# skim0119/gym-softrobot

Hardware: AMD Instinct MI355X
Metric: env_steps_per_sec (higher is better)
Workload: dtype f64

## Files before the change

### gym_softrobot_amd/_capi.py

```python
from __future__ import annotations

import ctypes as C
import os
from pathlib import Path

ABI_VERSION = 17

FEAT_GRAVITY = 1 << 0
FEAT_POINT_FORCE_NODE0_X = 1 << 1
FEAT_PENDULUM_BC = 1 << 2
FEAT_ANALYTICAL_DAMPER = 1 << 3
FEAT_FIXED_BC = 1 << 4
FEAT_TIP_FORCE = 1 << 5
FEAT_MOVING_BASE_BC = 1 << 6
FEAT_LAPLACE_FILTER = 1 << 7
FEAT_PLANE_CONTACT_ANISO = 1 << 8
FEAT_REST_KAPPA_ACTION = 1 << 9
FEAT_OCTO_HEAD = 1 << 10
FEAT_SPLINE_MUSCLE_TORQUES = 1 << 11
FEAT_SUCKER_CONSTRAINT = 1 << 12
FEAT_COOMM_MUSCLES = 1 << 13
MAX_SUCKERS = 4
MAX_MUSCLES = 4
MUSCLE_LONGITUDINAL = 0
# ... 893 lines not shown

_VP = C.c_void_p
_EXPORTS = {
    "softrod_abi_version": (C.c_int, []),
    "softrod_source_hash": (C.c_char_p, []),
    "softrod_action_dim": (C.c_int, [C.c_int]),
    "softrod_obs_dim": (C.c_int, [C.c_int]),
    "softrod_aux_dim": (C.c_int, [C.c_int]),
    "softrod_config_softpendulum": (C.c_int, [C.POINTER(SoftrodConfig), C.c_int]),
    "softrod_config_softpendulum3d": (C.c_int, [C.POINTER(SoftrodConfig), C.c_int]),
    "softrod_config_arm_single": (C.c_int, [C.POINTER(SoftrodConfig), C.c_int]),
    "softrod_config_octo_flat": (C.c_int, [C.POINTER(SoftrodConfig), C.c_int]),
    "softrod_config_soft_arm": (C.c_int, [C.POINTER(SoftrodConfig), C.c_int]),
    "softrod_config_arm_push": (C.c_int, [C.POINTER(SoftrodConfig), C.c_int, C.c_int]),
    "softrod_config_arm_pull_weight": (C.c_int, [C.POINTER(SoftrodConfig), C.c_int]),
    "softrod_config_muscle_octopus": (C.c_int, [C.POINTER(SoftrodConfig), C.c_int, C.c_int]),
    "softrod_set_muscle_layers": (C.c_int, [_VP, _VP, _VP]),
    "softrod_set_spline_table": (C.c_int, [_VP, _VP, _VP]),
    "softrod_config_action_dim": (C.c_int, [C.POINTER(SoftrodConfig)]),
    "softrod_config_obs_dim": (C.c_int, [C.POINTER(SoftrodConfig)]),
    "softrod_reset_octo": (C.c_int, [_VP, _VP, _VP, _VP, _VP, _VP]),
    "softrod_autoreset_enable": (C.c_int, [_VP, C.c_int]),
    "softrod_autoreset_same_step": (C.c_int, [_VP, C.c_int]),
    "softrod_final_view": (C.c_int, [_VP, C.POINTER(C.c_void_p), C.POINTER(C.c_void_p), C.POINTER(C.c_void_p)]),
    "softrod_queue_push": (C.c_int, [_VP, _VP, _VP, C.c_int, _VP]),
    "softrod_queue_push_straight": (C.c_int, [_VP, _VP, _VP, _VP, _VP, C.c_int, _VP]),
    "softrod_queue_push_octo": (C.c_int, [_VP, _VP, _VP, _VP, _VP, C.c_int, _VP]),
    "softrod_queue_status": (C.c_int, [_VP, _VP, _VP, _VP]),
    "softrod_queue_status_begin": (C.c_int, [_VP, _VP]),
    "softrod_queue_status_poll": (C.c_int, [_VP, C.c_int, _VP, _VP]),
    "softrod_queue_advance": (C.c_int, [_VP, _VP, _VP]),
    "softrod_set_action_basis": (C.c_int, [_VP, _VP]),
    "softrod_set_radius_profile": (C.c_int, [_VP, _VP]),
    "softrod_create": (C.c_int, [C.POINTER(SoftrodConfig), C.c_int, C.POINTER(C.c_void_p)]),
    "softrod_reset": (C.c_int, [_VP, _VP, _VP, _VP]),
    "softrod_reset_straight": (C.c_int, [_VP, _VP, _VP, _VP, _VP, _VP]),
    "softrod_step": (C.c_int, [_VP, _VP, _VP, _VP, _VP, _VP, _VP, _VP]),
    "softrod_step_packed": (C.c_int, [_VP, _VP, _VP, _VP, _VP]),
    "softrod_scatter_rows": (C.c_int, [_VP, _VP, _VP, C.c_int, C.c_int, C.c_int64, C.c_int64, C.c_uint32, _VP]),
    "softrod_exchange_alloc": (C.c_int, [C.c_int, C.c_uint64, C.POINTER(C.c_void_p), _VP, C.POINTER(C.c_int)]),
    "softrod_exchange_open": (C.c_int, [C.c_int, _VP, C.c_int, C.POINTER(C.c_void_p)]),
    "softrod_exchange_close": (C.c_int, [C.c_int, _VP]),
    "softrod_exchange_free": (C.c_int, [C.c_int, _VP]),
    "softrod_observe": (C.c_int, [_VP, _VP, _VP, _VP]),
    "softrod_rod_energies": (C.c_int, [_VP, _VP, _VP]),
    "softrod_ground_reaction": (C.c_int, [_VP, _VP, _VP]),
# ... 88 lines not shown
```

### gym_softrobot_amd/backend.py

```python
from __future__ import annotations

import ctypes as C
from typing import Dict, Optional, Tuple

import numpy as np
import torch

from . import _capi
from ._capi import LANE_STRIDE, SoftrodConfig, SoftrodStateView, check, load_library
from .diagnostics import (JointLoads, MuscleLoads, RodClearance, RodDynamics, RodStrains, joint_loads_views,
                          muscle_loads_views, rod_clearance_views, rod_dynamics_views, rod_strains_views)


class _DevArray:

    def __init__(self, ptr: int, shape, typestr: str, owner):
        self._owner = owner
        self.__cuda_array_interface__ = {
            "shape": tuple(shape),
            "typestr": typestr,
            "data": (int(ptr), False),
            "version": 2,
            "strides": None,
        }
# ... 232 lines not shown
        check(
            self._lib.softrod_reset_octo(
                self._h, pos.ctypes.data, dirs.ctypes.data, tg.ctypes.data,
                m.ctypes.data if m is not None else None, self._stream(),
            ),
            self._h,
        )

    def autoreset_enable(self, depth: int) -> None:
        check(self._lib.softrod_autoreset_enable(self._h, int(depth)), self._h)
        self.queue_depth = int(depth)

    def autoreset_same_step(self, on: bool = True) -> None:
        check(self._lib.softrod_autoreset_same_step(self._h, int(bool(on))), self._h)
        self.same_step = bool(on)
        if on and getattr(self, "final_obs", None) is None:
            fo, ft, fa = C.c_void_p(), C.c_void_p(), C.c_void_p()
            check(self._lib.softrod_final_view(self._h, C.byref(fo), C.byref(ft), C.byref(fa)), self._h)
            n = self.n_envs
            self.final_obs = torch.as_tensor(_DevArray(fo.value, (n, self.obs_dim), "<f4", self), device=self.device)
            self.final_time = torch.as_tensor(_DevArray(ft.value, (n,), "<f8", self), device=self.device)
            self.final_aux = torch.as_tensor(_DevArray(fa.value, (n,), "<f8", self), device=self.device)

    @staticmethod
    def _counts(counts, n):
        return np.ascontiguousarray(counts, dtype=np.int32).reshape(n)

    def queue_push(self, theta0, counts) -> None:
        th = np.ascontiguousarray(theta0, dtype=np.float64).reshape(self.n_envs, -1)
        c = self._counts(counts, self.n_envs)
        check(self._lib.softrod_queue_push(self._h, th.ctypes.data, c.ctypes.data, th.shape[1], self._stream()),
              self._h)

    def queue_push_straight(self, start, direction, normal, counts) -> None:
        arrs = [np.ascontiguousarray(v, dtype=np.float64).reshape(self.n_envs, -1, 3)
                for v in (start, direction, normal)]
        c = self._counts(counts, self.n_envs)
        check(self._lib.softrod_queue_push_straight(
            self._h, arrs[0].ctypes.data, arrs[1].ctypes.data, arrs[2].ctypes.data, c.ctypes.data,
            arrs[0].shape[1], self._stream()), self._h)

    def queue_push_octo(self, targets, counts) -> None:
        na = int(self.cfg.n_arm)
        tg = np.ascontiguousarray(targets, dtype=np.float64).reshape(self.n_envs, -1, 4 if self.is_mocto else 2)
        m = tg.shape[1]
        pos, dirs = self._arm_frames()
# ... 351 lines not shown
```

### gym_softrobot_amd/csrc/softrod_capi.hip

```cpp
#include <hip/hip_runtime.h>
#include <hip/hip_ext.h>

#include <cmath>
#include <cstdio>
#include <cstdlib>
#include <cstring>
#include <new>
#include <string>
#include <vector>

#include "softrod_kernels.hpp"
#include "softrod_dynamics_readout.hpp"
#include "softrod_copy_envs.hpp"
#include "softrod_shape.hpp"
#include "softrod_reset_shapes.hpp"

using namespace softrod;

template <class Row>
struct EnvTable {
    Row* dev = nullptr;
    Row* host = nullptr;
    hipEvent_t ev = nullptr;
    void release() {
// ... 36 lines not shown
    std::vector<hipEvent_t> ev_start, ev_stop;
    int timed = 0;
    hipEvent_t ev_reset = nullptr;
    int q_depth = 0;
    double* d_queue = nullptr;
    double* h_queue = nullptr;
    int* d_consumed = nullptr;
    int* d_produced = nullptr;
    int* d_underflow = nullptr;
    uint8_t* d_flags = nullptr;
    int* h_produced = nullptr;
    std::vector<int> seen_consumed;
    std::vector<int2> pending;
    double* h_stage = nullptr;
    int2* h_where = nullptr;
    double* d_stage = nullptr;
    int2* d_where = nullptr;
    size_t stage_cap = 0;
    int* h_status = nullptr;
    hipEvent_t ev_status = nullptr;
    bool status_pending = false;
    hipEvent_t ev_queue = nullptr;
    bool same_step = false;
    float* d_final_obs = nullptr;
    double* d_final_time = nullptr;
    double* d_final_aux = nullptr;
    int rs_count = 0;
    unsigned long long rs_seed = 0;
    double* d_rs_field[4] = {nullptr, nullptr, nullptr, nullptr};
    int* d_rs_index = nullptr;
    int* d_rs_episode = nullptr;
    uint8_t* d_rs_picked = nullptr;
    EnvTable<EnvMaterial> env_mat;
    EnvTable<EnvContact> env_contact;
    int2* d_pairs = nullptr;
    int2* h_pairs = nullptr;
    hipEvent_t ev_pairs = nullptr;
    std::vector<uint8_t> is_dst;
    std::string err;
};

namespace {

thread_local std::string g_err;

int fail(softrod_handle* h, int code, const std::string& msg) {
// ... 238 lines not shown
    }
    SR_HIP(h, hipGetLastError());
    return SOFTROD_OK;
}

enum : unsigned { kOptMuscles = SOFTROD_FEAT_COOMM_MUSCLES, kOptEarlyTerm = kFeatEarlyTerm, kOptEnvMaterial = kFeatEnvMaterial,
                  kOptEnvContact = kFeatEnvContact, kOptCompiledFor = kOptEarlyTerm | kOptEnvMaterial | kOptEnvContact };
constexpr int kAny = -1, kMoctoEnvs = -2;
constexpr unsigned kAnyFeatures = kRuntimeFeatures;
using StepKernel = void (*)(RodParams, StatePtrs, const float*, float*, double*, uint8_t*, uint8_t*, double*, int, int, int);
using OctoKernel = void (*)(RodParams, StatePtrs, const float*, float*, double*, uint8_t*, uint8_t*, int, int, int);
using WindowKernel = void (*)(RodParams, StatePtrs, const float*, int, int);

struct StepRow {
    unsigned feats;
    int env;
    int math, epl;
    int taper, zup;
    int nw_min, nw_max;
    bool windowed;
    unsigned needs, honours;
    StepKernel step; OctoKernel octo; WindowKernel window;
    int epb, waves;
    const char* label;
};

constexpr StepRow compiled_row(unsigned F, int env, int epl, int taper, int nw_min, int nw_max, const char* label) {
    const bool rt = F == kRuntimeFeatures;
    StepRow r{};
    r.feats = rt ? kAnyFeatures : F & ~(kFeatPlaneZup | kOptCompiledFor);
    r.env = env; r.math = SOFTROD_MATH_FAST; r.epl = epl; r.taper = taper; r.nw_min = nw_min; r.nw_max = nw_max;
    r.zup = rt ? kAny : (F & kFeatPlaneZup) != 0;
    r.needs = rt ? 0u : F & kOptCompiledFor;
    r.honours = rt ? 0u : F & (kOptCompiledFor | kOptMuscles);
    r.epb = 1; r.label = label;
    return r;
}
template <unsigned F, int E, int EPL, bool TAPER = false>
constexpr StepRow fast_row(const char* label) {
    StepRow r = compiled_row(F, E, EPL, TAPER, 1, 1, label);
    r.step = softrod_step_fast_kernel<F, E, EPL, TAPER>;
    return r;
}
template <unsigned F, int MAXW, int EPB>
constexpr StepRow octo_row(int env, int nw_min, int nw_max, const char* label) {
    StepRow r = compiled_row(F, env, 1, kAny, nw_min, nw_max, label);
    r.octo = softrod_octo_step_kernel<F, MAXW, EPB>;
    r.epb = EPB; r.waves = EPB == 1 ? 0 : MAXW * EPB;
    return r;
}
template <unsigned F, int RPB>
constexpr StepRow window_row(const char* label) {
    StepRow r = compiled_row(F, SOFTROD_ENV_ARM_SINGLE, 2, 0, 1, 1, label);
    r.window = softrod_step_window_kernel<F, RPB>;
    r.windowed = true; r.epb = RPB; r.waves = 2 * RPB;
    return r;
}
template <bool ET>
constexpr StepRow libm_row(unsigned feats, int env, int zup, int taper, unsigned honours) {
    StepRow r{};
    r.feats = feats; r.env = env; r.math = SOFTROD_MATH_LIBM; r.epl = 1; r.taper = taper; r.zup = zup;
    r.nw_min = r.nw_max = r.epb = 1;
    r.needs = ET ? kOptEarlyTerm : 0u; r.honours = r.needs | kOptMuscles | honours;
    r.step = softrod_step_libm_kernel<ET>;
// ... 105 lines not shown
               "and on SOFTROD_ENV_ARM_PULL_WEIGHT only; other feature mixes: SOFTROD_MATH_LIBM";
    if (opts & kOptEnvMaterial) return material_why_not(h);
    if (opts & kOptEnvContact) return contact_why_not(h);
    return nullptr;
}

struct StepChoice { const StepRow* row; const char* why; };
StepChoice select_step(const softrod_handle* h, int epilogue = 1, unsigned with = 0u) {
    const unsigned opts = active_options(h) | with;
    const int e = h->cfg.env_kind, zup = (h->P.features & kFeatPlaneZup) != 0;
    const bool windowed = h->window_refresh > 0 && epilogue;
    for (const StepRow& r : kStepRows)
        if (r.math == h->cfg.math_mode && (r.feats == kAnyFeatures || r.feats == h->cfg.features) &&
            (r.env == kAny || (r.env == kMoctoEnvs ? mocto_kind(e) : r.env == e)) && r.epl == h->epl &&
            (r.taper == kAny || r.taper == (int)h->tapered) && (r.zup == kAny || r.zup == zup) &&
            r.nw_min <= h->nw && h->nw <= r.nw_max && r.windowed == windowed &&
            (!r.window || r.epb == (h->window_paired ? 4 : 1)) && !(r.needs & ~opts) && !(opts & ~r.honours))
            return {&r, nullptr};
    const char* why = why_no_row(h, with);
    if (!why) why = why_no_row(h, opts);
    return {nullptr, why ? why : "no step kernel is compiled for this handle's feature set, env kind and options"};
}

template <int W, class Row, class Bad, class Build>
int set_env_table(softrod_handle* h, EnvTable<Row>& T, const Row*& slot, unsigned option, const char* what,
                  const double* values, const double (&own)[W], const uint8_t* mask, void* stream, Bad bad, Build build) {
    const StepChoice serves = select_step(h, 1, option);
    if (!serves.row) return fail(h, SOFTROD_EINVAL, serves.why);
    const size_t N = (size_t)h->cfg.n_envs;
    for (size_t i = 0; i < N; ++i) {
        if (mask && !mask[i]) continue;
        if (const char* why = bad(values + W * i)) return fail(h, SOFTROD_EINVAL, what + std::to_string(i) + why);
    }
    SR_ON_DEVICE(h);
    hipStream_t st = (hipStream_t)stream;
    if (!T.dev) {
        SR_HIP(h, hipMalloc((void**)&T.dev, N * sizeof(Row)));
        SR_HIP(h, hipHostMalloc((void**)&T.host, N * sizeof(Row), hipHostMallocDefault));
        SR_HIP(h, hipEventCreateWithFlags(&T.ev, hipEventDisableTiming));
        Row R0;
        build(own, R0);
        for (size_t i = 0; i < N; ++i) T.host[i] = R0;
        slot = T.dev;
        SR_HIP(h, hipMemcpy(h->d_state, &h->S, sizeof(StatePtrs), hipMemcpyHostToDevice));
    } else {
        SR_HIP(h, hipEventSynchronize(T.ev));
    }
    for (size_t i = 0; i < N; ++i)
        if (!mask || mask[i]) build(values + W * i, T.host[i]);
    SR_HIP(h, hipMemcpyAsync(T.dev, T.host, N * sizeof(Row), hipMemcpyHostToDevice, st));
    SR_HIP(h, hipEventRecord(T.ev, st));
    return SOFTROD_OK;
}

template <class K, class... A>
void launch_stamped(K kernel, const dim3& grid, const dim3& block, hipStream_t st, hipEvent_t t0, hipEvent_t t1, A... args) {
    if (t0 || t1) hipExtLaunchKernelGGL(kernel, grid, block, 0, st, t0, t1, 0, args...);
    else hipLaunchKernelGGL(kernel, grid, block, 0, st, args...);
}

int launch_step(softrod_handle* h, const float* actions, float* obs, double* reward,
                uint8_t* term, uint8_t* trunc, double* aux, int n_sub, int epilogue, int pack,
                hipStream_t st) {
    if (h->q_depth > 0 && epilogue && !h->same_step) {
        if (const int rc = launch_autoreset(h, obs, reward, term, trunc, aux, pack, st)) return rc;
        if (h->rs_count > 0)
            if (const int rc = launch_reset_shapes(h, kPickSkipped, nullptr, obs, term, trunc, aux, pack, st)) return rc;
    }
    if ((h->cfg.features & SOFTROD_FEAT_COOMM_MUSCLES) && h->cfg.math_mode == SOFTROD_MATH_FAST) {
        const bool push = h->cfg.env_kind == SOFTROD_ENV_ARM_PUSH || is_pull(h) || is_mocto(h);
        if (is_mocto(h) && (!h->tapered || !h->muscles_set || (h->cfg.env_kind == SOFTROD_ENV_ARM_TWO && !h->basis_set)))
            return fail(h, SOFTROD_EINVAL, "the muscle octopus needs softrod_set_radius_profile and softrod_set_muscle_layers "
                                           "(and SOFTROD_ENV_ARM_TWO softrod_set_action_basis) before it steps");
        if (push && !h->tapered)
            return fail(h, SOFTROD_EINVAL, "SOFTROD_ENV_ARM_PUSH (SOFTROD_MATH_FAST): call softrod_set_radius_profile first "
                                           "(the reference's arm is tapered, arm_push_env.py:160-179)");
        if (!push && h->tapered)
            return fail(h, SOFTROD_EINVAL, "a tapered muscle rod outside SOFTROD_ENV_ARM_PUSH runs under SOFTROD_MATH_LIBM only");
    }
    const StepChoice c = select_step(h, epilogue);
    if (!c.row) return fail(h, SOFTROD_EINVAL, c.why);
    const StepChoice after = c.row->windowed ? select_step(h, 0) : StepChoice{nullptr, nullptr};
    if (c.row->windowed && !after.row) return fail(h, SOFTROD_EINVAL, after.why);
    auto launch = [&](const StepRow& r, int n, int epi, hipEvent_t t0, hipEvent_t t1) {
        const dim3 grid((unsigned)((h->cfg.n_envs + r.epb - 1) / r.epb)), block(kLanes * (r.waves ? r.waves : h->nw));
        if (r.window) launch_stamped(r.window, grid, block, st, t0, t1, h->P, h->S, actions, n, h->window_refresh);
        else if (r.octo) launch_stamped(r.octo, grid, block, st, t0, t1, h->P, h->S, actions, obs, reward, term, trunc, n, epi, pack);
        else launch_stamped(r.step, grid, block, st, t0, t1, h->P, h->S, actions, obs, reward, term, trunc, aux, n, epi, pack);
    };
    const bool timing = h->timed < (int)h->ev_start.size();
    const hipEvent_t t0 = timing ? h->ev_start[h->timed] : nullptr, t1 = timing ? h->ev_stop[h->timed] : nullptr;
    const bool mocto = c.row->env == kMoctoEnvs;
    const bool action_first = mocto && epilogue && actions, epilogue_last = mocto && epilogue;
    const dim3 grid((unsigned)h->cfg.n_envs), block(kLanes * h->nw);
    if (action_first)
        launch_stamped(softrod_mocto_action_kernel, grid, block, st, t0, nullptr, h->P, h->S, actions, n_sub);
    launch(*c.row, n_sub, epilogue, action_first ? nullptr : t0, (after.row || epilogue_last) ? nullptr : t1);
    if (after.row) launch(*after.row, 0, 1, nullptr, epilogue_last ? nullptr : t1);
    if (epilogue_last)
        launch_stamped(softrod_mocto_epilogue_kernel, grid, block, st, nullptr, t1, h->P, h->S, obs, reward, term, trunc, 1, pack);
    SR_HIP(h, hipGetLastError());
    if (timing) ++h->timed;
    if (h->q_depth > 0 && epilogue && h->same_step) {
        if (const int rc = launch_autoreset_same_step(h, obs, aux, pack, st)) return rc;
        if (h->rs_count > 0)
            if (const int rc = launch_reset_shapes(h, kPickFinished, nullptr, obs, term, trunc, aux, pack, st)) return rc;
    }
    return SOFTROD_OK;
}

int upload_and_reset(softrod_handle* h, hipStream_t st, bool use_mask) {
    const size_t N = (size_t)h->cfg.n_envs;
    SR_HIP(h, hipMemcpyAsync(h->d_init, h->h_init, N * h->init_stride * sizeof(double), hipMemcpyHostToDevice, st));
    if (use_mask)
        SR_HIP(h, hipMemcpyAsync(h->d_mask, h->h_mask, N, hipMemcpyHostToDevice, st));
    ResetArgs A{h->d_init, use_mask ? h->d_mask : nullptr};
    if (is_octo(h)) {
        OctoResetArgs OA{h->d_init, h->d_init + N * (size_t)h->cfg.n_arm * 18, use_mask ? h->d_mask : nullptr};
        hipLaunchKernelGGL(softrod_octo_reset_kernel, dim3((unsigned)N), dim3(kLanes * h->nw), 0, st, h->P, h->S, OA);
    } else
// ... 720 lines not shown
        autoreset_release(h);
        h->err = why;
    }
    return rc;
}

int softrod_autoreset_same_step(softrod_handle* h, int on) {
    if (!h) return fail(h, SOFTROD_EINVAL, "null argument");
    if (!h->q_depth) return fail(h, SOFTROD_EINVAL, "call softrod_autoreset_enable first");
    SR_ON_DEVICE(h);
    if (on && !h->d_final_obs) {
        const size_t N = (size_t)h->cfg.n_envs;
        float* fo = nullptr;
        double *ft = nullptr, *fa = nullptr;
        SR_HIP(h, alloc_owned(h, fo, N * (size_t)softrod_config_obs_dim(&h->cfg) * sizeof(float)));
        SR_HIP(h, alloc_owned(h, ft, N * sizeof(double)));
        SR_HIP(h, alloc_owned(h, fa, N * sizeof(double)));
        h->d_final_obs = fo; h->d_final_time = ft; h->d_final_aux = fa;
    }
    h->same_step = on != 0;
    return SOFTROD_OK;
}

int softrod_final_view(softrod_handle* h, float** final_obs, double** final_time, double** final_aux) {
    if (!h || !final_obs || !final_time || !final_aux) return fail(h, SOFTROD_EINVAL, "null argument");
    if (!h->same_step) return fail(h, SOFTROD_EINVAL, "call softrod_autoreset_same_step first");
    *final_obs = h->d_final_obs;
    *final_time = h->d_final_time;
    *final_aux = h->d_final_aux;
    return SOFTROD_OK;
}

namespace {
int queue_begin(softrod_handle* h, const int32_t* counts, int max_count) {
    if (!h->q_depth) return fail(h, SOFTROD_EINVAL, "call softrod_autoreset_enable first");
    if (!counts || max_count < 0) return fail(h, SOFTROD_EINVAL, "bad argument");
    const int N = h->cfg.n_envs;
    for (int e = 0; e < N; ++e) {
        if (counts[e] < 0 || counts[e] > max_count) return fail(h, SOFTROD_EINVAL, "counts[e] out of range");
        if (h->h_produced[e] + counts[e] - h->seen_consumed[e] > h->q_depth)
            return fail(h, SOFTROD_EINVAL, "reset queue overflow: staged + new records exceed depth");
    }
    SR_HIP(h, hipEventSynchronize(h->ev_queue));
    return SOFTROD_OK;
}
double* queue_slot(softrod_handle* h, int e, int k) {
// ... 848 lines not shown
int softrod_last_kernel_ms(softrod_handle* h, float* ms) {
    if (!h || !ms) return fail(h, SOFTROD_EINVAL, "null argument");
    if (h->timed < 1) return fail(h, SOFTROD_EINVAL, "timing not enabled or no timed launch yet");
    SR_ON_DEVICE(h);
    SR_HIP(h, hipEventSynchronize(h->ev_stop[h->timed - 1]));
    SR_HIP(h, hipEventElapsedTime(ms, h->ev_start[h->timed - 1], h->ev_stop[h->timed - 1]));
    return SOFTROD_OK;
}

const char* softrod_last_error(softrod_handle* h) { return h ? h->err.c_str() : g_err.c_str(); }

const char* softrod_kernel_tier(softrod_handle* h) {
    if (!h) return "";
    const StepChoice c = select_step(h);
    std::string t = c.row ? c.row->label : std::string("none: ") + c.why;
    auto fill = [&t](const char* token, const std::string& with) {
        const size_t at = t.find(token);
        if (at != std::string::npos) t.replace(at, std::strlen(token), with);
    };
    fill("{waves}", std::to_string(h->nw) + (h->nw == 1 ? " wave" : " waves"));
    fill("{refresh}", std::to_string(h->window_refresh));
    if (c.row && c.row->windowed)
        if (const StepRow* after = select_step(h, 0).row) t += std::string(" + ") + after->label + " epilogue";
    if (h->env_mat.dev) t += ",env material";
    if (h->env_contact.dev) t += ",env contact";
    h->tier = t;
    return h->tier.c_str();
}

int softrod_destroy(softrod_handle* h) {
    if (!h) return SOFTROD_OK;
    DeviceGuard guard_(h->device);
    (void)hipDeviceSynchronize();
    autoreset_release(h);
    for (void* p : h->owned) (void)hipFree(p);
    for (double* p : h->d_rs_field) if (p) (void)hipFree(p);
    if (h->h_init) (void)hipHostFree(h->h_init);
    h->env_mat.release();
    h->env_contact.release();
    if (h->h_mask) (void)hipHostFree(h->h_mask);
    for (hipEvent_t e : h->ev_start) (void)hipEventDestroy(e);
    for (hipEvent_t e : h->ev_stop) (void)hipEventDestroy(e);
    if (h->ev_reset) (void)hipEventDestroy(h->ev_reset);
    if (h->h_pairs) (void)hipHostFree(h->h_pairs);
    if (h->ev_pairs) (void)hipEventDestroy(h->ev_pairs);
    delete h;
// ... 11 lines not shown
```

### gym_softrobot_amd/csrc/softrod_fast.hpp

```cpp
#pragma once

namespace softrod {

__device__ __forceinline__ bool wave_any(bool p) { return __builtin_amdgcn_ballot_w64(p) != 0ull; }
__device__ __forceinline__ bool wave_any_of(unsigned long long lanes, bool p) {
    return (__builtin_amdgcn_ballot_w64(p) & lanes) != 0ull;
}

__device__ __forceinline__ double horner(double g, double y, double c) {
    double d;
    asm("v_fma_f64 %0, %1, %2, %3" : "=v"(d) : "v"(g), "v"(y), "v"(c));
    return d;
}
__device__ __forceinline__ void fma_over(double& d, double a, double b, double c) {
    asm("v_fma_f64 %0, %1, %2, %3" : "+v"(d) : "v"(a), "v"(b), "v"(c));
}
__device__ __forceinline__ void fma_inplace_u(double& x, double m, double a) {
    asm("v_fma_f64 %0, %1, %0, %2" : "+v"(x) : "s"(m), "v"(a));
}

template <bool LEAN = true>
__device__ __forceinline__ void sinc_cosc(double t, double& sc, double& cc) {
    if (!wave_any(t >= 1.0e-3)) {
        if constexpr (LEAN) {
// ... 453 lines not shown
    const double tb = P.time_two_half_adds ? P.half_dt : 0.0;
    for (int s = 0; s < n_sub; ++s) time = (time + ta) + tb;
    return time;
}

template <unsigned F, int EPL, bool TAPER = false>
__device__ __forceinline__ void general_substeps(const RodParams& P, const RodParams& Pk, const ConstN<EPL>& C,
                                                 const BcTargets& B, int lane, LaneN<EPL>& L, int n_sub) {
#if SOFTROD_IDLE_LANES_EXEC_MASK
    if (has<F>(P, SOFTROD_FEAT_SPLINE_MUSCLE_TORQUES) || slot_local<F>(P, lane * EPL) <= P.n_elem)
#endif
    {
        kinematic_n<EPL>(P.half_dt, C, L);
        ProgressPriority prio(n_sub);
        for (int s = 0; s < n_sub; ++s) {
            dynamic_n<F, EPL, TAPER>(Pk, C, B, lane, L);
            const bool last = (s == n_sub - 1);
            kinematic_n<EPL>(last ? P.half_dt : P.dt, C, L);
            prio.tick(s);
        }
    }
}
template <unsigned F, int E, int EPL>
__device__ __attribute__((noinline)) void general_step_cold(const RodParams* __restrict__ params,
                                                            const StatePtrs* __restrict__ sp, int rod, int lane,
                                                            const float* __restrict__ actions, int n_sub, int poison) {
    const RodParams P = *params;
    const StatePtrs S = *sp;
    const size_t N = (size_t)P.n_envs;
    LaneN<EPL> L;
    double time;
    if (poison) {
        poison_rod<EPL>(L);
        time = S.time[rod];
    } else {
        load_lane<EPL, F>(S, N, rod, lane, L);
        BcTargets B;
        load_bc(S, N, rod, B);
        EnvAction A;
        set_action_n<F, E, EPL>(P, S, N, rod, lane, actions, A, B, L);
        constrain_rates_n<F, EPL>(P, B, lane, L);
        constrain_values_n<F, EPL>(P, B, lane, L);
        time = S.time[rod];
        if (n_sub > 0) {
            ConstN<EPL> C;
            if constexpr (kEnvMaterial<F>) build_const_m<F, EPL>(P, S.env_mat[rod], lane, A, C);
            else build_const<F, EPL>(P, lane, A, C);
            if constexpr (kEnvContact<F>) C.ct = S.env_contact[rod];
            RodParams Pk = P;
            if (!has<F>(P, SOFTROD_FEAT_ANALYTICAL_DAMPER)) Pk.damp_t = 1.0;
            general_substeps<F, EPL>(P, Pk, C, B, lane, L, n_sub);
        }
    }
    time = clock_after(P, S, time, n_sub);
    store_lane<EPL, F>(S, N, rod, lane, L);
    if (lane == 0) S.time[rod] = time;
}

#ifndef SOFTROD_FAST_WAVES
#define SOFTROD_FAST_WAVES 3
#endif
#ifndef SOFTROD_PLANAR_WAVES
#define SOFTROD_PLANAR_WAVES 4
#endif
#ifndef SOFTROD_PLANAR_EXEC_MASK
#define SOFTROD_PLANAR_EXEC_MASK 1
#endif
#ifndef SOFTROD_CONTACT_WAVES
#define SOFTROD_CONTACT_WAVES 2
#endif
#ifndef SOFTROD_RUNTIME_WAVES
#define SOFTROD_RUNTIME_WAVES 2
#endif
#ifdef SOFTROD_PHASE_CLOCKS
__device__ unsigned long long g_phase_clock[16384][8];
#define SR_PHASE(i) do { __builtin_amdgcn_s_waitcnt(0); if (threadIdx.x == 0 && blockIdx.x < 16384) \
        g_phase_clock[blockIdx.x][i] = wall_clock64(); } while (0)
#else
#define SR_PHASE(i) do {} while (0)
#endif

// ... 1 lines not shown
constexpr int fast_kernel_waves() {
    if (EPL > 1) return 1;
    if (F == kRuntimeFeatures) return SOFTROD_RUNTIME_WAVES;
    if (F & (SOFTROD_FEAT_PLANE_CONTACT_ANISO | SOFTROD_FEAT_LAPLACE_FILTER | SOFTROD_FEAT_SPLINE_MUSCLE_TORQUES |
             SOFTROD_FEAT_COOMM_MUSCLES))
        return SOFTROD_CONTACT_WAVES;
    if (TAPER) return SOFTROD_CONTACT_WAVES;
    return (F & ~kFeatEnvMaterial) == SOFTROD_FEATURES_SOFTPENDULUM ? SOFTROD_PLANAR_WAVES : SOFTROD_FAST_WAVES;
}

template <unsigned F, int E, int EPL, bool TAPER = false>
__global__ void __launch_bounds__(kLanes, (fast_kernel_waves<F, EPL, TAPER>()))
softrod_step_fast_kernel(const RodParams P, const StatePtrs S, const float* __restrict__ actions,
                         float* __restrict__ obs, double* __restrict__ reward,
                         uint8_t* __restrict__ terminated, uint8_t* __restrict__ truncated,
                         double* __restrict__ aux, const int n_sub, const int epilogue, const int pack) {
    const int rod = blockIdx.x;
    const int lane = threadIdx.x;
    const size_t N = (size_t)P.n_envs;
    [[maybe_unused]] EnvMaterial M;
    if constexpr (kEnvMaterial<F>) M = S.env_mat[rod];
    [[maybe_unused]] EnvContact CT;
    if constexpr (kEnvContact<F>) CT = S.env_contact[rod];
    if (epilogue && S.skip && S.skip[rod]) {
        if (lane == 0) S.skip[rod] = 0;
        if (lane == 0 && early_term_on<F>(P)) S.aux[rod] = 0.0;
        return;
    }

    __builtin_amdgcn_s_setprio(3);
    SR_PHASE(0);
    constexpr bool kPlanarKernel = (F & ~kFeatEnvMaterial) == SOFTROD_FEATURES_SOFTPENDULUM;
    LaneN<EPL> L;
    load_lane<EPL, F, !kPlanarKernel>(S, N, rod, lane, L);
    SR_PHASE(1);
    if (has<F>(P, SOFTROD_FEAT_LAPLACE_FILTER)) sanitize_unused_rates<EPL>(P, lane, L);
    if (has<F>(P, SOFTROD_FEAT_PLANE_CONTACT_ANISO)) sanitize_unused_slots<EPL>(P, lane, L);
    BcTargets B;
    load_bc(S, N, rod, B);
    load_suckers<F>(P, S, N, rod, B);
    EnvAction A;
    set_action_n<F, E, EPL>(P, S, N, rod, lane, actions, A, B, L);
    if (epilogue) push_store_prev_com<F, E, EPL>(P, S, N, rod, lane, L, n_sub);
    if (has<F>(P, SOFTROD_FEAT_SPLINE_MUSCLE_TORQUES)) muscle_load<EPL>(P, S, rod, actions != nullptr, A, L);
    {
        BcTargets B0 = B;
        if (has<F>(P, SOFTROD_FEAT_MOVING_BASE_BC)) {
            B0.vel[0] = __shfl(L.v[0][0], 0); B0.vel[1] = __shfl(L.v[0][1], 0); B0.vel[2] = __shfl(L.v[0][2], 0);
        }
        constrain_rates_n<F, EPL>(P, B0, lane, L);
        constrain_values_n<F, EPL>(P, B, lane, L);
    }
    double time = S.time[rod];
    ConstN<EPL> C;
    if constexpr (kEnvMaterial<F>) build_const_m<F, EPL, TAPER>(P, M, lane, A, C, S.mat);
    else build_const_m<F, EPL, TAPER>(P, P, lane, A, C, S.mat);
    if constexpr (kEnvContact<F>) C.ct = CT;
    if constexpr (kMusclesCompiled<F>) build_muscle_const<F, EPL, true>(P, S, N, rod, lane, A, C);
    RodParams Pk = P;
    if (!has<F>(P, SOFTROD_FEAT_ANALYTICAL_DAMPER)) Pk.damp_t = 1.0;

    bool blown_up = false;
    if (n_sub > 0 && epilogue && rod_has_nan<EPL>(P, lane, L)) {
        blown_up = true;
        if constexpr (!kPlanarKernel) {
            poison_rod<EPL>(L);
            time = clock_after(P, S, time, n_sub);
        }
    }
    if constexpr (kPlanarKernel) {
        PlanarN<EPL> Z;
        if (n_sub > 0 && !blown_up && planar_from_lane<EPL>(P, B, lane, L, Z)) {
            PlanarC<EPL> K;
            planar_build_const<EPL, kEnvMaterial<F>>(Pk, C, lane, K);
            const double ta = P.time_two_half_adds ? P.half_dt : P.dt;
            const double tb = P.time_two_half_adds ? P.half_dt : 0.0;
            int tk = -1;
            if (S.time_tab && n_sub == P.tab_n_sub) {
                const double kf = rint(time * P.inv_step_time);
                const int k = (kf >= 0.0 && kf < (double)(P.tab_len - 1)) ? (int)kf : -1;
                tk = (k >= 0 && S.time_tab[k] == time) ? k : -1;
            }
            const double step_dt = EPL > 1 ? opaque_v(P.dt) : P.dt;
            SR_PHASE(2);
#if SOFTROD_PLANAR_EXEC_MASK
            if (lane * EPL <= P.n_elem) {
#endif
                planar_kinematic_n<EPL>(P.half_dt, K.hq_hdt, C, K, Z);
                {
                    int s = 0;
#pragma unroll
                    for (int q = 0; q < 4; ++q) {
                        if (q == 1) __builtin_amdgcn_s_setprio(2);
                        if (q == 2) __builtin_amdgcn_s_setprio(1);
                        if (q == 3) __builtin_amdgcn_s_setprio(0);
// ... 8 lines not shown
#endif
                        }
                    }
                }
                planar_dynamic_n<EPL>(Pk, C, K, lane, Z);
                planar_kinematic_n<EPL>(P.half_dt, K.hq_hdt, C, K, Z);
#if SOFTROD_PLANAR_EXEC_MASK
            }
#endif
            if (__builtin_amdgcn_readfirstlane(tk) >= 0) time = S.time_tab[tk + 1];
            else
                for (int s = 0; s < n_sub; ++s) time = (time + ta) + tb;
            SR_PHASE(3);
            planar_store<EPL>(S, N, rod, lane, Z, !SOFTROD_PLANAR_EXEC_MASK || lane * EPL <= P.n_elem);
#pragma unroll
            for (int s = 0; s < EPL; ++s) {
#pragma unroll
                for (int c = 0; c < 3; ++c) { L.x[s][c] = 0.0; L.v[s][c] = 0.0; L.w[s][c] = 0.0; L.t[s][c] = 0.0; }
#pragma unroll
                for (int c = 0; c < 9; ++c) L.Q[s][c] = 0.0;
            }
            planar_to_lane<EPL>(Z, L);
        } else {
            general_step_cold<F, E, EPL>(S.params, S.self, rod, lane, actions, n_sub, blown_up);
            __builtin_amdgcn_fence(__ATOMIC_ACQUIRE, "wavefront");
            load_lane<EPL, F>(S, N, rod, opaque_lane(lane), L);
            time = S.time[rod];
        }
    } else {
        if (n_sub > 0 && !blown_up) {
            general_substeps<F, EPL, TAPER>(P, Pk, C, B, lane, L, n_sub);
            time = clock_after(P, S, time, n_sub);
        }
        store_lane<EPL, F>(S, N, rod, lane, L);
    }
    if (has<F>(P, SOFTROD_FEAT_SPLINE_MUSCLE_TORQUES)) muscle_store<EPL>(P, S, rod, lane, L);
    if (env_of<E>(P) == SOFTROD_ENV_SOFT_ARM && lane == 0)
        S.ctrl[(size_t)0 * N + rod] += (double)n_sub;
    if (lane == 0) S.time[rod] = time;
    SR_PHASE(4);
    if (epilogue)
        env_epilogue_n<E, EPL, F>(P, S, N, rod, lane, C, L, time, A, obs, reward, terminated, truncated, aux, pack);
    SR_PHASE(5);
}


}
// ... 1 lines not shown
```

### gym_softrobot_amd/csrc/softrod_kernels.hpp

```cpp
#pragma once
#include <hip/hip_runtime.h>
#include <stdint.h>

#include "../../include/softrod.h"

namespace softrod {

constexpr int kLanes = 64;

constexpr unsigned kRuntimeFeatures = 0xFFFFFFFFu;
constexpr unsigned kFeaturesTaperedSuckerArm = SOFTROD_FEAT_ANALYTICAL_DAMPER | SOFTROD_FEAT_SUCKER_CONSTRAINT;
constexpr unsigned kFeatPlaneZup = 1u << 30;
constexpr unsigned kFeatEarlyTerm = 1u << 29;
constexpr unsigned kFeatEnvMaterial = 1u << 28;
template <unsigned F>
constexpr bool kEnvMaterial = F != kRuntimeFeatures && (F & kFeatEnvMaterial) != 0;
constexpr unsigned kFeatEnvContact = 1u << 27;
template <unsigned F>
constexpr bool kEnvContact = F != kRuntimeFeatures && (F & kFeatEnvContact) != 0;
constexpr int kRuntimeEnv = -1;
constexpr unsigned kFeaturesMuscleRod = SOFTROD_FEAT_FIXED_BC | SOFTROD_FEAT_ANALYTICAL_DAMPER | SOFTROD_FEAT_COOMM_MUSCLES;
template <unsigned F>
constexpr bool kMusclesCompiled = F != kRuntimeFeatures && (F & SOFTROD_FEAT_COOMM_MUSCLES) != 0;

// ... 1775 lines not shown



template <int EPL>
__global__ void __launch_bounds__(kLanes)
softrod_reset_kernel(const RodParams P, const StatePtrs S, const ResetArgs A) {
    const int rod = blockIdx.x;
    if (A.mask && !A.mask[rod]) return;
    LaneN<EPL> L;
    reset_rod<EPL>(P, S, (size_t)P.n_envs, rod, threadIdx.x, A.init + (size_t)rod * 18, L);
}

__global__ void __launch_bounds__(kLanes)
softrod_queue_scatter_kernel(double* __restrict__ queue, const double* __restrict__ staged,
                             const int2* __restrict__ where, const int n_envs, const int record) {
    const int m = blockIdx.x;
    const int2 w = where[m];
    double* dst = queue + ((size_t)w.y * (size_t)n_envs + (size_t)w.x) * (size_t)record;
    const double* src = staged + (size_t)m * (size_t)record;
    for (int i = threadIdx.x; i < record; i += kLanes) dst[i] = src[i];
}

template <int EPL>
__global__ void __launch_bounds__(kLanes)
softrod_autoreset_kernel(const RodParams P, const StatePtrs S, float* __restrict__ obs,
                         double* __restrict__ reward, uint8_t* __restrict__ terminated,
                         uint8_t* __restrict__ truncated, double* __restrict__ aux, const int pack) {
    const int rod = blockIdx.x;
    const int lane = threadIdx.x;
    if (!S.needs_reset[rod]) return;
    const size_t N = (size_t)P.n_envs;
    const int k = S.q_consumed[rod];
    if (k >= S.q_produced[rod]) {
        if (lane == 0) atomicAdd(S.q_underflow, 1);
        return;
    }
    const double* in = S.queue + ((size_t)(k % S.q_depth) * N + rod) * (size_t)S.q_record;
    LaneN<EPL> L;
    reset_rod<EPL>(P, S, N, rod, lane, in, L);
    EnvAction A;
#pragma unroll
    for (int i = 0; i < 7; ++i) A.a[i] = 0.0f;
    A.force = 0.0;
    A.mu_set = false;
    ConstN<EPL> C;
    const EnvMaterial E = env_material_rt(P, S, rod);
    if (S.mat) build_const_m<kRuntimeFeatures, EPL, true>(P, E, lane, A, C, S.mat);
    else build_const_m<kRuntimeFeatures, EPL>(P, E, lane, A, C);
    float pa[7];
#pragma unroll
    for (int i = 0; i < 7; ++i) pa[i] = S.prev_action[7 * (size_t)rod + i];
    const int od = env_obs_dim(P);
    float* o = out_row(obs, rod, od, pack);
    env_observe_n<kRuntimeEnv, EPL>(P, S, N, rod, lane, C, L, pa, o);
    if (lane == 0) {
        emit_scalars(o, od, pack, rod, 0.0, false, false, reward, terminated, truncated, S.needs_reset);
        if (aux && P.env_kind == SOFTROD_ENV_SOFTPENDULUM3D) aux[rod] = (double)o[8];
        S.skip[rod] = 1;
        S.q_consumed[rod] = k + 1;
    }
}

}

#include "softrod_fast.hpp"
#include "softrod_octo.hpp"
#include "softrod_window.hpp"
#include "softrod_literal.hpp"
#include "softrod_readout.hpp"
#include "softrod_reaction.hpp"
#include "softrod_strains.hpp"
#include "softrod_muscle_readout.hpp"
#include "softrod_joint_readout.hpp"
#include "softrod_render.hpp"
#include "softrod_clearance.hpp"
#include "softrod_autoreset.hpp"
```

### include/softrod.h

```cpp
#ifndef SOFTROD_H
#define SOFTROD_H

#include <stddef.h>
#include <stdint.h>

#ifdef __cplusplus
extern "C" {
#endif

#define SOFTROD_ABI_VERSION 17

#define SOFTROD_OK 0
#define SOFTROD_EINVAL (-1)
#define SOFTROD_ENOMEM (-2)
#define SOFTROD_EHIP (-3)
#define SOFTROD_ENODEV (-4)

enum softrod_feature {
    SOFTROD_FEAT_GRAVITY = 1u << 0,
    SOFTROD_FEAT_POINT_FORCE_NODE0_X = 1u << 1,
    SOFTROD_FEAT_PENDULUM_BC = 1u << 2,
    SOFTROD_FEAT_ANALYTICAL_DAMPER = 1u << 3,
    SOFTROD_FEAT_FIXED_BC = 1u << 4,
    SOFTROD_FEAT_TIP_FORCE = 1u << 5,
// ... 177 lines not shown

int softrod_create(const softrod_config* cfg, int device, softrod_handle** out);

int softrod_reset(softrod_handle* h, const double* theta0, const uint8_t* mask,
                  void* stream);

int softrod_reset_straight(softrod_handle* h, const double* start,
                           const double* direction, const double* normal,
                           const uint8_t* mask, void* stream);

int softrod_reset_octo(softrod_handle* h, const double* arm_start,
                       const double* arm_direction, const double* target,
                       const uint8_t* mask, void* stream);

int softrod_step(softrod_handle* h, const float* actions, float* obs,
                 double* reward, uint8_t* terminated, uint8_t* truncated,
                 double* aux, void* stream);

int softrod_step_packed(softrod_handle* h, const float* actions, float* packed,
                        double* aux, void* stream);

int softrod_autoreset_enable(softrod_handle* h, int depth);
int softrod_autoreset_same_step(softrod_handle* h, int on);
int softrod_final_view(softrod_handle* h, float** final_obs, double** final_time, double** final_aux);
int softrod_queue_push(softrod_handle* h, const double* theta0, const int32_t* counts,
                       int max_count, void* stream);
int softrod_queue_push_straight(softrod_handle* h, const double* start,
                                const double* direction, const double* normal,
                                const int32_t* counts, int max_count, void* stream);
int softrod_queue_push_octo(softrod_handle* h, const double* arm_start,
                            const double* arm_direction, const double* target,
                            const int32_t* counts, int max_count, void* stream);
int softrod_queue_status(softrod_handle* h, int32_t* consumed, int32_t* underflow,
                         void* stream);
int softrod_queue_status_begin(softrod_handle* h, void* stream);
int softrod_queue_status_poll(softrod_handle* h, int wait, int32_t* consumed, int32_t* underflow);
int softrod_queue_advance(softrod_handle* h, const int32_t* by, void* stream);

#define SOFTROD_MAX_PEERS 16
int softrod_scatter_rows(softrod_handle* h, const float* packed, const uint64_t* peer_buffers,
                         int n_peers, int row_words, int64_t first_row, int64_t tag_word,
                         uint32_t tag, void* stream);

#define SOFTROD_IPC_HANDLE_BYTES 64
#define SOFTROD_EXCHANGE_UNCACHED 1
#define SOFTROD_EXCHANGE_FINEGRAINED 2
// ... 77 lines not shown
```

Measured before the change: 14.26 million.

## Fuse queued auto-reset into the fast step kernel

Moves the per-rod auto-reset into the fast step kernel: rods that need a reset pop their queued initial state inside the step launch, which replaces the separate autoreset kernel launch before each step. The autoreset body is factored into a shared device function. Resetting rods now return early rather than being flagged with skip and handled on the next step. The intent is to remove one kernel launch and an extra pass over all rods per step, at the cost of more code (and possible register pressure) in the hot kernel and different skip semantics.

```diff
diff --git a/gym_softrobot_amd/_capi.py b/gym_softrobot_amd/_capi.py
--- a/gym_softrobot_amd/_capi.py
+++ b/gym_softrobot_amd/_capi.py
@@ -939,6 +939,9 @@
     "softrod_reset_octo": (C.c_int, [_VP, _VP, _VP, _VP, _VP, _VP]),
     "softrod_autoreset_enable": (C.c_int, [_VP, C.c_int]),
     "softrod_autoreset_same_step": (C.c_int, [_VP, C.c_int]),
+    "softrod_set_fused_autoreset": (C.c_int, [_VP, C.c_int]),
+    "softrod_config_fused_autoreset": (C.c_int, [C.POINTER(SoftrodConfig), C.c_int, C.c_int, C.c_int, C.c_int]),
+    "softrod_autoreset_flags_view": (C.c_int, [_VP, C.POINTER(C.c_void_p), C.POINTER(C.c_void_p)]),
     "softrod_final_view": (C.c_int, [_VP, C.POINTER(C.c_void_p), C.POINTER(C.c_void_p), C.POINTER(C.c_void_p)]),
     "softrod_queue_push": (C.c_int, [_VP, _VP, _VP, C.c_int, _VP]),
     "softrod_queue_push_straight": (C.c_int, [_VP, _VP, _VP, _VP, _VP, C.c_int, _VP]),
diff --git a/gym_softrobot_amd/backend.py b/gym_softrobot_amd/backend.py
--- a/gym_softrobot_amd/backend.py
+++ b/gym_softrobot_amd/backend.py
@@ -278,6 +278,14 @@
             self.final_time = torch.as_tensor(_DevArray(ft.value, (n,), "<f8", self), device=self.device)
             self.final_aux = torch.as_tensor(_DevArray(fa.value, (n,), "<f8", self), device=self.device)
 
+    def set_fused_autoreset(self, on: bool = True) -> None:
+        check(self._lib.softrod_set_fused_autoreset(self._h, int(bool(on))), self._h)
+
+    def autoreset_flags(self):
+        nr, sk = C.c_void_p(), C.c_void_p()
+        check(self._lib.softrod_autoreset_flags_view(self._h, C.byref(nr), C.byref(sk)), self._h)
+        return tuple(torch.as_tensor(_DevArray(p.value, (self.n_envs,), "|u1", self), device=self.device) for p in (nr, sk))
+
     @staticmethod
     def _counts(counts, n):
         return np.ascontiguousarray(counts, dtype=np.int32).reshape(n)
diff --git a/gym_softrobot_amd/csrc/softrod_capi.hip b/gym_softrobot_amd/csrc/softrod_capi.hip
--- a/gym_softrobot_amd/csrc/softrod_capi.hip
+++ b/gym_softrobot_amd/csrc/softrod_capi.hip
@@ -82,6 +82,7 @@
     bool status_pending = false;
     hipEvent_t ev_queue = nullptr;
     bool same_step = false;
+    bool fused_autoreset = true;
     float* d_final_obs = nullptr;
     double* d_final_time = nullptr;
     double* d_final_aux = nullptr;
@@ -366,6 +367,7 @@
     unsigned needs, honours;
     StepKernel step; OctoKernel octo; WindowKernel window;
     int epb, waves;
+    bool fused_autoreset;
     const char* label;
 };
 
@@ -384,6 +386,7 @@
 constexpr StepRow fast_row(const char* label) {
     StepRow r = compiled_row(F, E, EPL, TAPER, 1, 1, label);
     r.step = softrod_step_fast_kernel<F, E, EPL, TAPER>;
+    r.fused_autoreset = kFusedAutoreset<F, E>;
     return r;
 }
 template <unsigned F, int MAXW, int EPB>
@@ -535,6 +538,11 @@
     return {nullptr, why ? why : "no step kernel is compiled for this handle's feature set, env kind and options"};
 }
 
+bool fuses_autoreset(const softrod_handle* h, const StepRow* row) {
+    return row && row->fused_autoreset && !row->windowed && h->window_refresh == 0 && h->q_depth > 0 && !h->same_step &&
+           h->rs_count == 0 && h->fused_autoreset && h->cfg.env_kind != SOFTROD_ENV_ARM_PUSH;
+}
+
 template <int W, class Row, class Bad, class Build>
 int set_env_table(softrod_handle* h, EnvTable<Row>& T, const Row*& slot, unsigned option, const char* what,
                   const double* values, const double (&own)[W], const uint8_t* mask, void* stream, Bad bad, Build build) {
@@ -575,7 +583,8 @@
 int launch_step(softrod_handle* h, const float* actions, float* obs, double* reward,
                 uint8_t* term, uint8_t* trunc, double* aux, int n_sub, int epilogue, int pack,
                 hipStream_t st) {
-    if (h->q_depth > 0 && epilogue && !h->same_step) {
+    const bool fused = epilogue && fuses_autoreset(h, select_step(h, epilogue).row);
+    if (h->q_depth > 0 && epilogue && !h->same_step && !fused) {
         if (const int rc = launch_autoreset(h, obs, reward, term, trunc, aux, pack, st)) return rc;
         if (h->rs_count > 0)
             if (const int rc = launch_reset_shapes(h, kPickSkipped, nullptr, obs, term, trunc, aux, pack, st)) return rc;
@@ -608,7 +617,7 @@
     const dim3 grid((unsigned)h->cfg.n_envs), block(kLanes * h->nw);
     if (action_first)
         launch_stamped(softrod_mocto_action_kernel, grid, block, st, t0, nullptr, h->P, h->S, actions, n_sub);
-    launch(*c.row, n_sub, epilogue, action_first ? nullptr : t0, (after.row || epilogue_last) ? nullptr : t1);
+    launch(*c.row, n_sub, fused ? epilogue | kEpilogueFusedAutoreset : epilogue, action_first ? nullptr : t0, (after.row || epilogue_last) ? nullptr : t1);
     if (after.row) launch(*after.row, 0, 1, nullptr, epilogue_last ? nullptr : t1);
     if (epilogue_last)
         launch_stamped(softrod_mocto_epilogue_kernel, grid, block, st, nullptr, t1, h->P, h->S, obs, reward, term, trunc, 1, pack);
@@ -1375,6 +1384,35 @@
     return SOFTROD_OK;
 }
 
+int softrod_set_fused_autoreset(softrod_handle* h, int on) {
+    if (!h) return fail(h, SOFTROD_EINVAL, "null argument");
+    h->fused_autoreset = on != 0;
+    return SOFTROD_OK;
+}
+
+int softrod_config_fused_autoreset(const softrod_config* cfg, int tapered, int same_step, int reset_shapes, int fused) {
+    if (!cfg) return fail(nullptr, SOFTROD_EINVAL, "null argument");
+    if (cfg->struct_size != sizeof(softrod_config)) return fail(nullptr, SOFTROD_EINVAL, "softrod_config.struct_size mismatch");
+    if (const char* why = config_why_not(*cfg)) return fail(nullptr, SOFTROD_EINVAL, why);
+    softrod_handle h;
+    h.cfg = *cfg;
+    shape_handle(&h);
+    h.tapered = tapered != 0;
+    h.q_depth = 1;
+    h.same_step = same_step != 0;
+    h.rs_count = reset_shapes != 0;
+    h.fused_autoreset = fused != 0;
+    return fuses_autoreset(&h, select_step(&h).row) ? 1 : 0;
+}
+
+int softrod_autoreset_flags_view(softrod_handle* h, uint8_t** needs_reset, uint8_t** skip) {
+    if (!h || !needs_reset || !skip) return fail(h, SOFTROD_EINVAL, "null argument");
+    if (!h->q_depth) return fail(h, SOFTROD_EINVAL, "call softrod_autoreset_enable first");
+    *needs_reset = h->S.needs_reset;
+    *skip = h->S.skip;
+    return SOFTROD_OK;
+}
+
 int softrod_final_view(softrod_handle* h, float** final_obs, double** final_time, double** final_aux) {
     if (!h || !final_obs || !final_time || !final_aux) return fail(h, SOFTROD_EINVAL, "null argument");
     if (!h->same_step) return fail(h, SOFTROD_EINVAL, "call softrod_autoreset_same_step first");
@@ -2269,6 +2307,7 @@
     fill("{refresh}", std::to_string(h->window_refresh));
     if (c.row && c.row->windowed)
         if (const StepRow* after = select_step(h, 0).row) t += std::string(" + ") + after->label + " epilogue";
+    if (fuses_autoreset(h, c.row)) t += ",fused auto-reset";
     if (h->env_mat.dev) t += ",env material";
     if (h->env_contact.dev) t += ",env contact";
     h->tier = t;
diff --git a/gym_softrobot_amd/csrc/softrod_fast.hpp b/gym_softrobot_amd/csrc/softrod_fast.hpp
--- a/gym_softrobot_amd/csrc/softrod_fast.hpp
+++ b/gym_softrobot_amd/csrc/softrod_fast.hpp
@@ -499,12 +499,20 @@
     }
 }
 template <unsigned F, int E, int EPL>
-__device__ __attribute__((noinline)) void general_step_cold(const RodParams* __restrict__ params,
+__device__ __attribute__((noinline, cold)) void general_step_cold(const RodParams* __restrict__ params,
                                                             const StatePtrs* __restrict__ sp, int rod, int lane,
-                                                            const float* __restrict__ actions, int n_sub, int poison) {
+                                                            const float* __restrict__ actions, int n_sub, int poison,
+                                                            int restart, float* __restrict__ obs,
+                                                            double* __restrict__ reward, uint8_t* __restrict__ terminated,
+                                                            uint8_t* __restrict__ truncated, double* __restrict__ aux,
+                                                            int pack) {
     const RodParams P = *params;
     const StatePtrs S = *sp;
     const size_t N = (size_t)P.n_envs;
+    if (restart >= 0) {
+        autoreset_rod<EPL>(P, S, rod, lane, restart, obs, reward, terminated, truncated, aux, pack, false);
+        return;
+    }
     LaneN<EPL> L;
     double time;
     if (poison) {
@@ -534,6 +542,30 @@
     if (lane == 0) S.time[rod] = time;
 }
 
+template <unsigned F, int E>
+constexpr bool kFusedAutoreset = E != SOFTROD_ENV_ARM_PUSH && E != SOFTROD_ENV_NONE &&
+                                 (F == kRuntimeFeatures || !(F & SOFTROD_FEAT_COOMM_MUSCLES));
+constexpr int kEpilogueFusedAutoreset = 2;
+__device__ __forceinline__ int staged_restart(const StatePtrs& S, int rod, int lane, int epilogue) {
+    int restart = -1;
+    if (__builtin_expect((epilogue & kEpilogueFusedAutoreset) && S.needs_reset[rod], 0)) {
+        const int k = S.q_consumed[rod];
+        if (k < S.q_produced[rod]) restart = k;
+        else if (lane == 0) atomicAdd(S.q_underflow, 1);
+    }
+    return restart;
+}
+template <int EPL>
+__device__ __attribute__((noinline)) void autoreset_cold(const RodParams* __restrict__ params,
+                                                         const StatePtrs* __restrict__ sp, int rod, int lane, int restart,
+                                                         float* __restrict__ obs, double* __restrict__ reward,
+                                                         uint8_t* __restrict__ terminated, uint8_t* __restrict__ truncated,
+                                                         double* __restrict__ aux, int pack) {
+    const RodParams P = *params;
+    const StatePtrs S = *sp;
+    autoreset_rod<EPL>(P, S, rod, lane, restart, obs, reward, terminated, truncated, aux, pack, false);
+}
+
 #ifndef SOFTROD_FAST_WAVES
 #define SOFTROD_FAST_WAVES 3
 #endif
@@ -581,55 +613,69 @@
     if constexpr (kEnvMaterial<F>) M = S.env_mat[rod];
     [[maybe_unused]] EnvContact CT;
     if constexpr (kEnvContact<F>) CT = S.env_contact[rod];
-    if (epilogue && S.skip && S.skip[rod]) {
+    constexpr bool kPlanarKernel = (F & ~kFeatEnvMaterial) == SOFTROD_FEATURES_SOFTPENDULUM;
+    int restart = -1;
+    if constexpr (kFusedAutoreset<F, E>) {
+        restart = staged_restart(S, rod, lane, epilogue);
+        if constexpr (!kPlanarKernel) {
+            if (__builtin_expect(restart >= 0, 0)) {
+                autoreset_cold<EPL>(S.params, S.self, rod, opaque_lane(lane), restart, obs, reward, terminated, truncated, aux,
+                                    pack);
+                return;
+            }
+        }
+    }
+    if (epilogue == 1 && S.skip && S.skip[rod]) {
         if (lane == 0) S.skip[rod] = 0;
         if (lane == 0 && early_term_on<F>(P)) S.aux[rod] = 0.0;
         return;
     }
 
-    __builtin_amdgcn_s_setprio(3);
-    SR_PHASE(0);
-    constexpr bool kPlanarKernel = (F & ~kFeatEnvMaterial) == SOFTROD_FEATURES_SOFTPENDULUM;
     LaneN<EPL> L;
-    load_lane<EPL, F, !kPlanarKernel>(S, N, rod, lane, L);
-    SR_PHASE(1);
-    if (has<F>(P, SOFTROD_FEAT_LAPLACE_FILTER)) sanitize_unused_rates<EPL>(P, lane, L);
-    if (has<F>(P, SOFTROD_FEAT_PLANE_CONTACT_ANISO)) sanitize_unused_slots<EPL>(P, lane, L);
     BcTargets B;
-    load_bc(S, N, rod, B);
-    load_suckers<F>(P, S, N, rod, B);
     EnvAction A;
-    set_action_n<F, E, EPL>(P, S, N, rod, lane, actions, A, B, L);
-    if (epilogue) push_store_prev_com<F, E, EPL>(P, S, N, rod, lane, L, n_sub);
-    if (has<F>(P, SOFTROD_FEAT_SPLINE_MUSCLE_TORQUES)) muscle_load<EPL>(P, S, rod, actions != nullptr, A, L);
-    {
-        BcTargets B0 = B;
-        if (has<F>(P, SOFTROD_FEAT_MOVING_BASE_BC)) {
-            B0.vel[0] = __shfl(L.v[0][0], 0); B0.vel[1] = __shfl(L.v[0][1], 0); B0.vel[2] = __shfl(L.v[0][2], 0);
-        }
-        constrain_rates_n<F, EPL>(P, B0, lane, L);
-        constrain_values_n<F, EPL>(P, B, lane, L);
-    }
-    double time = S.time[rod];
+    double time = 0.0;
     ConstN<EPL> C;
-    if constexpr (kEnvMaterial<F>) build_const_m<F, EPL, TAPER>(P, M, lane, A, C, S.mat);
-    else build_const_m<F, EPL, TAPER>(P, P, lane, A, C, S.mat);
-    if constexpr (kEnvContact<F>) C.ct = CT;
-    if constexpr (kMusclesCompiled<F>) build_muscle_const<F, EPL, true>(P, S, N, rod, lane, A, C);
     RodParams Pk = P;
     if (!has<F>(P, SOFTROD_FEAT_ANALYTICAL_DAMPER)) Pk.damp_t = 1.0;
-
     bool blown_up = false;
-    if (n_sub > 0 && epilogue && rod_has_nan<EPL>(P, lane, L)) {
-        blown_up = true;
-        if constexpr (!kPlanarKernel) {
-            poison_rod<EPL>(L);
-            time = clock_after(P, S, time, n_sub);
+    if (__builtin_expect(restart < 0, 1)) {
+        __builtin_amdgcn_s_setprio(3);
+        SR_PHASE(0);
+        load_lane<EPL, F, !kPlanarKernel>(S, N, rod, lane, L);
+        SR_PHASE(1);
+        if (has<F>(P, SOFTROD_FEAT_LAPLACE_FILTER)) sanitize_unused_rates<EPL>(P, lane, L);
+        if (has<F>(P, SOFTROD_FEAT_PLANE_CONTACT_ANISO)) sanitize_unused_slots<EPL>(P, lane, L);
+        load_bc(S, N, rod, B);
+        load_suckers<F>(P, S, N, rod, B);
+        set_action_n<F, E, EPL>(P, S, N, rod, lane, actions, A, B, L);
+        if (epilogue) push_store_prev_com<F, E, EPL>(P, S, N, rod, lane, L, n_sub);
+        if (has<F>(P, SOFTROD_FEAT_SPLINE_MUSCLE_TORQUES)) muscle_load<EPL>(P, S, rod, actions != nullptr, A, L);
+        {
+            BcTargets B0 = B;
+            if (has<F>(P, SOFTROD_FEAT_MOVING_BASE_BC)) {
+                B0.vel[0] = __shfl(L.v[0][0], 0); B0.vel[1] = __shfl(L.v[0][1], 0); B0.vel[2] = __shfl(L.v[0][2], 0);
+            }
+            constrain_rates_n<F, EPL>(P, B0, lane, L);
+            constrain_values_n<F, EPL>(P, B, lane, L);
+        }
+        time = S.time[rod];
+        if constexpr (kEnvMaterial<F>) build_const_m<F, EPL, TAPER>(P, M, lane, A, C, S.mat);
+        else build_const_m<F, EPL, TAPER>(P, P, lane, A, C, S.mat);
+        if constexpr (kEnvContact<F>) C.ct = CT;
+        if constexpr (kMusclesCompiled<F>) build_muscle_const<F, EPL, true>(P, S, N, rod, lane, A, C);
+
+        if (n_sub > 0 && epilogue && rod_has_nan<EPL>(P, lane, L)) {
+            blown_up = true;
+            if constexpr (!kPlanarKernel) {
+                poison_rod<EPL>(L);
+                time = clock_after(P, S, time, n_sub);
+            }
         }
     }
     if constexpr (kPlanarKernel) {
         PlanarN<EPL> Z;
-        if (n_sub > 0 && !blown_up && planar_from_lane<EPL>(P, B, lane, L, Z)) {
+        if (__builtin_expect(restart < 0, 1) && n_sub > 0 && !blown_up && planar_from_lane<EPL>(P, B, lane, L, Z)) {
             PlanarC<EPL> K;
             planar_build_const<EPL, kEnvMaterial<F>>(Pk, C, lane, K);
             const double ta = P.time_two_half_adds ? P.half_dt : P.dt;
@@ -684,7 +730,9 @@
             }
             planar_to_lane<EPL>(Z, L);
         } else {
-            general_step_cold<F, E, EPL>(S.params, S.self, rod, lane, actions, n_sub, blown_up);
+            general_step_cold<F, E, EPL>(S.params, S.self, rod, lane, actions, n_sub, blown_up, restart, obs, reward,
+                                         terminated, truncated, aux, pack);
+            if (restart >= 0) return;
             __builtin_amdgcn_fence(__ATOMIC_ACQUIRE, "wavefront");
             load_lane<EPL, F>(S, N, rod, opaque_lane(lane), L);
             time = S.time[rod];
diff --git a/gym_softrobot_amd/csrc/softrod_kernels.hpp b/gym_softrobot_amd/csrc/softrod_kernels.hpp
--- a/gym_softrobot_amd/csrc/softrod_kernels.hpp
+++ b/gym_softrobot_amd/csrc/softrod_kernels.hpp
@@ -1821,19 +1821,11 @@
 }
 
 template <int EPL>
-__global__ void __launch_bounds__(kLanes)
-softrod_autoreset_kernel(const RodParams P, const StatePtrs S, float* __restrict__ obs,
-                         double* __restrict__ reward, uint8_t* __restrict__ terminated,
-                         uint8_t* __restrict__ truncated, double* __restrict__ aux, const int pack) {
-    const int rod = blockIdx.x;
-    const int lane = threadIdx.x;
-    if (!S.needs_reset[rod]) return;
+__device__ __forceinline__ void autoreset_rod(const RodParams& P, const StatePtrs& S, const int rod, const int lane, const int k,
+                                              float* __restrict__ obs, double* __restrict__ reward,
+                                              uint8_t* __restrict__ terminated, uint8_t* __restrict__ truncated,
+                                              double* __restrict__ aux, const int pack, const bool mark_skip) {
     const size_t N = (size_t)P.n_envs;
-    const int k = S.q_consumed[rod];
-    if (k >= S.q_produced[rod]) {
-        if (lane == 0) atomicAdd(S.q_underflow, 1);
-        return;
-    }
     const double* in = S.queue + ((size_t)(k % S.q_depth) * N + rod) * (size_t)S.q_record;
     LaneN<EPL> L;
     reset_rod<EPL>(P, S, N, rod, lane, in, L);
@@ -1855,9 +1847,25 @@
     if (lane == 0) {
         emit_scalars(o, od, pack, rod, 0.0, false, false, reward, terminated, truncated, S.needs_reset);
         if (aux && P.env_kind == SOFTROD_ENV_SOFTPENDULUM3D) aux[rod] = (double)o[8];
-        S.skip[rod] = 1;
+        if (mark_skip) S.skip[rod] = 1;
         S.q_consumed[rod] = k + 1;
     }
+}
+
+template <int EPL>
+__global__ void __launch_bounds__(kLanes)
+softrod_autoreset_kernel(const RodParams P, const StatePtrs S, float* __restrict__ obs,
+                         double* __restrict__ reward, uint8_t* __restrict__ terminated,
+                         uint8_t* __restrict__ truncated, double* __restrict__ aux, const int pack) {
+    const int rod = blockIdx.x;
+    const int lane = threadIdx.x;
+    if (!S.needs_reset[rod]) return;
+    const int k = S.q_consumed[rod];
+    if (k >= S.q_produced[rod]) {
+        if (lane == 0) atomicAdd(S.q_underflow, 1);
+        return;
+    }
+    autoreset_rod<EPL>(P, S, rod, lane, k, obs, reward, terminated, truncated, aux, pack, true);
 }
 
 }
diff --git a/include/softrod.h b/include/softrod.h
--- a/include/softrod.h
+++ b/include/softrod.h
@@ -223,6 +223,9 @@
 
 int softrod_autoreset_enable(softrod_handle* h, int depth);
 int softrod_autoreset_same_step(softrod_handle* h, int on);
+int softrod_set_fused_autoreset(softrod_handle* h, int on);
+int softrod_config_fused_autoreset(const softrod_config* cfg, int tapered, int same_step, int reset_shapes, int fused);
+int softrod_autoreset_flags_view(softrod_handle* h, uint8_t** needs_reset, uint8_t** skip);
 int softrod_final_view(softrod_handle* h, float** final_obs, double** final_time, double** final_aux);
 int softrod_queue_push(softrod_handle* h, const double* theta0, const int32_t* counts,
                        int max_count, void* stream);
```

After: 14.17 million. Within noise of the previous version (-0.6%).
